# HKUST-KnowComp/DummyNode4GraphLearning

Hardware: AMD Instinct MI355X
Metric: edges/sec fwd+bwd on dummy-augmented RGIN conv (higher is better)
Workload: dtype bf16; 1 GPU; config5: RGINLayer(256,256,R=16,basis,relu) fwd+bwd, ONE global batch of 32768 graphs cut by parallel.shard_graphs over 1 GPU(s) (rank 0: N=1015808, E=3997696), SI dummy augmentation; global_edges=3997696, parallelism=dp1, rows_P=3112960, grad_bucket_bytes=2491904, hip_graph=True, sub_batches=1

## Files before the change

dummynode4graphlearning_amd/csrc/dn_chain_wgrad.hip:

```cpp
#include "dn_common.h"
#include "dn_internal.h"
#include "../../include/dn_hip.h"

namespace {

typedef __bf16 bf16_t;

constexpr int kH = 256;
constexpr int kTile = 64;
constexpr int kKC = 32;
constexpr int kThreads = 256;
constexpr int kAld = kTile + 2;

__device__ __forceinline__ double bf16_to_f64(bf16_t v) { return (double)(float)v; }

__device__ __forceinline__ bf16_t f64_to_bf16(double d) {
    float f = (float)d;
    if ((double)f != d && f == f && fabsf(f) < __builtin_huge_valf()) {
        uint32_t u = __float_as_uint(f);
        if (fabs((double)f) > fabs(d)) u -= 1u;
        f = __uint_as_float(u | 1u);
    }
    return (bf16_t)f;
}

__global__ __launch_bounds__(kThreads) void chain_combine_products_kernel(const float* __restrict__ M, const bf16_t* __restrict__ W1,
                                                                          const bf16_t* __restrict__ Wc,
                                                                          const bf16_t* __restrict__ Wc_loop, int32_t R,
                                                                          bf16_t* __restrict__ dWc, double* __restrict__ part) {
    __shared__ __attribute__((aligned(16))) double As[kKC * kAld];
    __shared__ __attribute__((aligned(16))) double Bs[kKC * kTile];
    const int tid = threadIdx.x, ty = tid >> 4, tx = tid & 15;
    const int m0 = (int)(blockIdx.x >> 2) * kTile, n0 = (int)(blockIdx.x & 3) * kTile;
    const int r = (int)blockIdx.y, kind = (int)blockIdx.z;
    const float* Mr = M + (size_t)r * kH * kH;
    const bf16_t* B = kind == 0 ? W1 : (r < R ? Wc + (size_t)r * kH * kH : Wc_loop);
    double acc[4][4];
#pragma unroll
    for (int i = 0; i < 4; ++i)
#pragma unroll
        for (int j = 0; j < 4; ++j) acc[i][j] = 0.0;
    float ra[8];
    bf16_t rb[8];
    auto fetch = [&](int kc) __attribute__((always_inline)) {
#pragma unroll
        for (int s = 0; s < 8; ++s) {
            if (kind == 0) ra[s] = Mr[(size_t)(m0 + (tid >> 5) + 8 * s) * kH + kc + (tid & 31)];
            else ra[s] = Mr[(size_t)(kc + (tid >> 6) + 4 * s) * kH + m0 + (tid & 63)];
            rb[s] = B[(size_t)(kc + (tid >> 6) + 4 * s) * kH + n0 + (tid & 63)];
        }
    };
    fetch(0);
    for (int kc = 0; kc < kH; kc += kKC) {
#pragma unroll
        for (int s = 0; s < 8; ++s) {
            if (kind == 0) As[(tid & 31) * kAld + (tid >> 5) + 8 * s] = (double)ra[s];
            else As[((tid >> 6) + 4 * s) * kAld + (tid & 63)] = (double)ra[s];
            Bs[((tid >> 6) + 4 * s) * kTile + (tid & 63)] = bf16_to_f64(rb[s]);
        }
        if (kc + kKC < kH) fetch(kc + kKC);
        __syncthreads();
#pragma unroll 8
        for (int k = 0; k < kKC; ++k) {
            const double2 a01 = *reinterpret_cast<const double2*>(&As[k * kAld + 4 * ty]);
            const double2 a23 = *reinterpret_cast<const double2*>(&As[k * kAld + 4 * ty + 2]);
            const double2 b01 = *reinterpret_cast<const double2*>(&Bs[k * kTile + 4 * tx]);
            const double2 b23 = *reinterpret_cast<const double2*>(&Bs[k * kTile + 4 * tx + 2]);
            const double a[4] = {a01.x, a01.y, a23.x, a23.y}, b[4] = {b01.x, b01.y, b23.x, b23.y};
#pragma unroll
            for (int i = 0; i < 4; ++i)
#pragma unroll
                for (int j = 0; j < 4; ++j) acc[i][j] = fma(a[i], b[j], acc[i][j]);
        }
        __syncthreads();
    }
#pragma unroll
    for (int i = 0; i < 4; ++i)
#pragma unroll
        for (int j = 0; j < 4; ++j) {
            const size_t o = (size_t)r * kH * kH + (size_t)(m0 + 4 * ty + i) * kH + n0 + 4 * tx + j;
            if (kind == 0) dWc[o] = f64_to_bf16(acc[i][j]);
            else part[o] = acc[i][j];
        }
}

__global__ __launch_bounds__(kH) void chain_combine_finish_kernel(const double* __restrict__ part, const float* __restrict__ c,
                                                                  const bf16_t* __restrict__ W1, const bf16_t* __restrict__ bias,
                                                                  int32_t R, bf16_t* __restrict__ dW1, bf16_t* __restrict__ db,
                                                                  bf16_t* __restrict__ db1) {
    const int h = threadIdx.x, j = (int)blockIdx.x;
    if (j < kH) {
        double sum = 0.0;
        for (int r = 0; r <= R; ++r) sum += part[(size_t)r * kH * kH + (size_t)j * kH + h];
        if (bias) sum = fma((double)c[j], bf16_to_f64(bias[h]), sum);
        dW1[(size_t)j * kH + h] = f64_to_bf16(sum);
        return;
    }
    if (db) {
        double sum = 0.0;
        for (int jj = 0; jj < kH; ++jj) sum = fma((double)c[jj], bf16_to_f64(W1[(size_t)jj * kH + h]), sum);
        db[h] = f64_to_bf16(sum);
    }
    if (db1) db1[h] = (bf16_t)c[h];
}

}

extern "C" int dn_layer_chain_dgrad_bf16(const void* G1, const void* W_kn, int64_t N, int32_t H, const int32_t* tiles, int64_t num_tiles,
                                         void* G0, void* seg_sums, dn_stream_t stream) {
    DN_REQUIRE(H == 256, "dn_layer_chain_dgrad: unsupported width %d (256 only)", H);
    DN_REQUIRE(N >= 0 && N < 0x7fffffffLL && num_tiles >= 0 && num_tiles < 0x7fffffffLL, "dn_layer_chain_dgrad: bad sizes");
    if (num_tiles == 0) return DN_OK;
    DN_REQUIRE(G1 && W_kn && tiles && G0 && seg_sums, "dn_layer_chain_dgrad: NULL pointer");
    DN_REQUIRE((reinterpret_cast<uintptr_t>(G1) | reinterpret_cast<uintptr_t>(W_kn) | reinterpret_cast<uintptr_t>(tiles) |
                reinterpret_cast<uintptr_t>(G0) | reinterpret_cast<uintptr_t>(seg_sums)) % 16 == 0, "dn_layer_chain_dgrad: unaligned pointer");
    return dn_internal::launch_transform_ring256_seg(G1, W_kn, tiles, num_tiles, G0, seg_sums, (hipStream_t)stream);
}

extern "C" size_t dn_layer_chain_wgrad_combine_workspace_bytes(int64_t R, int32_t H) {
    return R >= 0 && H > 0 ? (size_t)(R + 1) * (size_t)H * (size_t)H * sizeof(double) : 0;
}

extern "C" int dn_layer_chain_wgrad_combine(const float* M, const float* c, const void* W1, const void* Wc, const void* Wc_loop,
                                            const void* bias, int64_t R, int32_t H, void* dWc, void* db, void* dW1, void* db1,
                                            void* workspace, size_t workspace_bytes, dn_stream_t stream) {
    DN_REQUIRE(H == 256, "dn_layer_chain_wgrad_combine: unsupported width %d (256 only)", H);
    DN_REQUIRE(R >= 0 && R < 65535, "dn_layer_chain_wgrad_combine: bad relation count");
    DN_REQUIRE(M && c && W1 && Wc_loop && dWc && dW1 && workspace && (Wc || R == 0), "dn_layer_chain_wgrad_combine: NULL pointer");
    DN_REQUIRE(workspace_bytes >= dn_layer_chain_wgrad_combine_workspace_bytes(R, H), "dn_layer_chain_wgrad_combine: workspace too small");
    DN_REQUIRE((reinterpret_cast<uintptr_t>(M) | reinterpret_cast<uintptr_t>(workspace)) % 16 == 0,
               "dn_layer_chain_wgrad_combine: unaligned pointer");
    hipStream_t st = (hipStream_t)stream;
    double* part = (double*)workspace;
    hipLaunchKernelGGL(chain_combine_products_kernel, dim3((kH / kTile) * (kH / kTile), (unsigned)(R + 1), 2), dim3(kThreads), 0, st, M,
                       (const bf16_t*)W1, (const bf16_t*)Wc, (const bf16_t*)Wc_loop, (int32_t)R, (bf16_t*)dWc, part);
    DN_CHECK_LAUNCH();
    hipLaunchKernelGGL(chain_combine_finish_kernel, dim3(kH + 1), dim3(kH), 0, st, (const double*)part, c, (const bf16_t*)W1,
                       (const bf16_t*)bias, (int32_t)R, (bf16_t*)dW1, (bf16_t*)db, (bf16_t*)db1);
    DN_CHECK_LAUNCH();
    return DN_OK;
}
```

Before: 1.398 billion edges/s.

## Fuse chain wgrad combine into one FP64 MFMA kernel without workspace

```diff
diff --git a/dummynode4graphlearning_amd/csrc/dn_chain_wgrad.hip b/dummynode4graphlearning_amd/csrc/dn_chain_wgrad.hip
--- a/dummynode4graphlearning_amd/csrc/dn_chain_wgrad.hip
+++ b/dummynode4graphlearning_amd/csrc/dn_chain_wgrad.hip
@@ -7,10 +7,12 @@
 typedef __bf16 bf16_t;
 
 constexpr int kH = 256;
-constexpr int kTile = 64;
-constexpr int kKC = 32;
+constexpr int kT = 16;
 constexpr int kThreads = 256;
-constexpr int kAld = kTile + 2;
+constexpr int kW1Blocks = (kH / kT) * (kH / kT);
+constexpr int kWcBlocksPerRel = (kH / kT) * (kH / (4 * kT));
+
+typedef double f64x4 __attribute__((ext_vector_type(4)));
 
 __device__ __forceinline__ double bf16_to_f64(bf16_t v) { return (double)(float)v; }
 
@@ -24,81 +26,116 @@
     return (bf16_t)f;
 }
 
-__global__ __launch_bounds__(kThreads) void chain_combine_products_kernel(const float* __restrict__ M, const bf16_t* __restrict__ W1,
-                                                                          const bf16_t* __restrict__ Wc,
-                                                                          const bf16_t* __restrict__ Wc_loop, int32_t R,
-                                                                          bf16_t* __restrict__ dWc, double* __restrict__ part) {
-    __shared__ __attribute__((aligned(16))) double As[kKC * kAld];
-    __shared__ __attribute__((aligned(16))) double Bs[kKC * kTile];
-    const int tid = threadIdx.x, ty = tid >> 4, tx = tid & 15;
-    const int m0 = (int)(blockIdx.x >> 2) * kTile, n0 = (int)(blockIdx.x & 3) * kTile;
-    const int r = (int)blockIdx.y, kind = (int)blockIdx.z;
-    const float* Mr = M + (size_t)r * kH * kH;
-    const bf16_t* B = kind == 0 ? W1 : (r < R ? Wc + (size_t)r * kH * kH : Wc_loop);
-    double acc[4][4];
+__device__ __forceinline__ f64x4 mfma_f64(double a, double b, f64x4 acc) { return __builtin_amdgcn_mfma_f64_16x16x4f64(a, b, acc, 0, 0, 0); }
+
+constexpr int kU = 8;
+
+__device__ __forceinline__ f64x4 chain_rows(const float* __restrict__ Ap, const bf16_t* __restrict__ Bp, int steps, f64x4 acc) {
+    float a0[kU], a1[kU];
+    bf16_t b0[kU], b1[kU];
+    auto load = [&](float (&a)[kU], bf16_t (&b)[kU], int s) __attribute__((always_inline)) {
 #pragma unroll
-    for (int i = 0; i < 4; ++i)
-#pragma unroll
-        for (int j = 0; j < 4; ++j) acc[i][j] = 0.0;
-    float ra[8];
-    bf16_t rb[8];
-    auto fetch = [&](int kc) __attribute__((always_inline)) {
-#pragma unroll
-        for (int s = 0; s < 8; ++s) {
-            if (kind == 0) ra[s] = Mr[(size_t)(m0 + (tid >> 5) + 8 * s) * kH + kc + (tid & 31)];
-            else ra[s] = Mr[(size_t)(kc + (tid >> 6) + 4 * s) * kH + m0 + (tid & 63)];
-            rb[s] = B[(size_t)(kc + (tid >> 6) + 4 * s) * kH + n0 + (tid & 63)];
+        for (int u = 0; u < kU; ++u) {
+            a[u] = Ap[(size_t)(s + u) * 4 * kH];
+            b[u] = Bp[(size_t)(s + u) * 4 * kH];
         }
     };
-    fetch(0);
-    for (int kc = 0; kc < kH; kc += kKC) {
+    auto mma = [&](const float (&a)[kU], const bf16_t (&b)[kU]) __attribute__((always_inline)) {
 #pragma unroll
-        for (int s = 0; s < 8; ++s) {
-            if (kind == 0) As[(tid & 31) * kAld + (tid >> 5) + 8 * s] = (double)ra[s];
-            else As[((tid >> 6) + 4 * s) * kAld + (tid & 63)] = (double)ra[s];
-            Bs[((tid >> 6) + 4 * s) * kTile + (tid & 63)] = bf16_to_f64(rb[s]);
-        }
-        if (kc + kKC < kH) fetch(kc + kKC);
-        __syncthreads();
-#pragma unroll 8
-        for (int k = 0; k < kKC; ++k) {
-            const double2 a01 = *reinterpret_cast<const double2*>(&As[k * kAld + 4 * ty]);
-            const double2 a23 = *reinterpret_cast<const double2*>(&As[k * kAld + 4 * ty + 2]);
-            const double2 b01 = *reinterpret_cast<const double2*>(&Bs[k * kTile + 4 * tx]);
-            const double2 b23 = *reinterpret_cast<const double2*>(&Bs[k * kTile + 4 * tx + 2]);
-            const double a[4] = {a01.x, a01.y, a23.x, a23.y}, b[4] = {b01.x, b01.y, b23.x, b23.y};
-#pragma unroll
-            for (int i = 0; i < 4; ++i)
-#pragma unroll
-                for (int j = 0; j < 4; ++j) acc[i][j] = fma(a[i], b[j], acc[i][j]);
-        }
-        __syncthreads();
+        for (int u = 0; u < kU; ++u) acc = mfma_f64((double)a[u], bf16_to_f64(b[u]), acc);
+    };
+    if (steps <= 0) return acc;
+    load(a0, b0, 0);
+    for (int s = 0; s < steps; s += 2 * kU) {
+        load(a1, b1, s + kU);
+        mma(a0, b0);
+        if (s + 2 * kU < steps) load(a0, b0, s + 2 * kU);
+        mma(a1, b1);
     }
-#pragma unroll
-    for (int i = 0; i < 4; ++i)
-#pragma unroll
-        for (int j = 0; j < 4; ++j) {
-            const size_t o = (size_t)r * kH * kH + (size_t)(m0 + 4 * ty + i) * kH + n0 + 4 * tx + j;
-            if (kind == 0) dWc[o] = f64_to_bf16(acc[i][j]);
-            else part[o] = acc[i][j];
-        }
+    return acc;
 }
 
-__global__ __launch_bounds__(kH) void chain_combine_finish_kernel(const double* __restrict__ part, const float* __restrict__ c,
-                                                                  const bf16_t* __restrict__ W1, const bf16_t* __restrict__ bias,
-                                                                  int32_t R, bf16_t* __restrict__ dW1, bf16_t* __restrict__ db,
-                                                                  bf16_t* __restrict__ db1) {
-    const int h = threadIdx.x, j = (int)blockIdx.x;
-    if (j < kH) {
-        double sum = 0.0;
-        for (int r = 0; r <= R; ++r) sum += part[(size_t)r * kH * kH + (size_t)j * kH + h];
-        if (bias) sum = fma((double)c[j], bf16_to_f64(bias[h]), sum);
-        dW1[(size_t)j * kH + h] = f64_to_bf16(sum);
+__global__ __launch_bounds__(kThreads) void chain_combine_mfma_kernel(const float* __restrict__ M, const float* __restrict__ c,
+                                                                      const bf16_t* __restrict__ W1, const bf16_t* __restrict__ Wc,
+                                                                      const bf16_t* __restrict__ Wc_loop, const bf16_t* __restrict__ bias,
+                                                                      int32_t R, bf16_t* __restrict__ dWc, bf16_t* __restrict__ db,
+                                                                      bf16_t* __restrict__ dW1, bf16_t* __restrict__ db1) {
+    __shared__ double red[3][4][64];
+    const int tid = threadIdx.x, lane = tid & 63, wave = tid >> 6, li = lane & 15, lk = lane >> 4;
+    const int b = (int)blockIdx.x;
+    if (b < kW1Blocks) {
+        const int m0 = (2 * (b & 7) + ((b >> 3) & 1)) * kT, n0 = (b >> 4) * kT;
+        const int rows = (R + 1) * (kH / 4), row0 = wave * rows, loop0 = R * kH;
+        const int rows_wc = min(max(loop0 - row0, 0), rows);
+        const float* Ap = M + (size_t)(row0 + lk) * kH + m0 + li;
+        f64x4 acc = {0.0, 0.0, 0.0, 0.0};
+        if (rows_wc > 0) acc = chain_rows(Ap, Wc + (size_t)(row0 + lk) * kH + n0 + li, rows_wc / 4, acc);
+        if (rows_wc < rows)
+            acc = chain_rows(Ap + (size_t)rows_wc * kH, Wc_loop + (size_t)(row0 + rows_wc - loop0 + lk) * kH + n0 + li, (rows - rows_wc) / 4, acc);
+        if (wave)
+#pragma unroll
+            for (int v = 0; v < 4; ++v) red[wave - 1][v][lane] = acc[v];
+        __syncthreads();
+        if (wave) return;
+#pragma unroll
+        for (int v = 0; v < 4; ++v) {
+            const int j = m0 + lk + 4 * v, h = n0 + li;
+            double sum = ((acc[v] + red[0][v][lane]) + red[1][v][lane]) + red[2][v][lane];
+            if (bias) sum = fma((double)c[j], bf16_to_f64(bias[h]), sum);
+            dW1[(size_t)j * kH + h] = f64_to_bf16(sum);
+        }
         return;
     }
+    const int t = b - kW1Blocks;
+    if (t < (R + 1) * kWcBlocksPerRel) {
+        const int id = (t >> 5) * 8 + (t & 7), r = id >> 4, m0 = (id & 15) * kT, n0 = ((t >> 3) & 3) * 4 * kT + wave * kT;
+        const float* Ap = M + ((size_t)r * kH + m0 + li) * kH + 4 * lk;
+        const bf16_t* Bp = W1 + (size_t)(4 * lk) * kH + n0 + li;
+        f64x4 acc = {0.0, 0.0, 0.0, 0.0};
+        float4 a0[2], a1[2];
+        bf16_t b0[2][4], b1[2][4];
+        auto load = [&](float4 (&a)[2], bf16_t (&bb)[2][4], int kc) __attribute__((always_inline)) {
+#pragma unroll
+            for (int u = 0; u < 2; ++u) {
+                a[u] = *reinterpret_cast<const float4*>(Ap + kc + 16 * u);
+#pragma unroll
+                for (int s = 0; s < 4; ++s) bb[u][s] = Bp[(size_t)(kc + 16 * u + s) * kH];
+            }
+        };
+        auto mma = [&](const float4 (&a)[2], const bf16_t (&bb)[2][4]) __attribute__((always_inline)) {
+#pragma unroll
+            for (int u = 0; u < 2; ++u) {
+                acc = mfma_f64((double)a[u].x, bf16_to_f64(bb[u][0]), acc);
+                acc = mfma_f64((double)a[u].y, bf16_to_f64(bb[u][1]), acc);
+                acc = mfma_f64((double)a[u].z, bf16_to_f64(bb[u][2]), acc);
+                acc = mfma_f64((double)a[u].w, bf16_to_f64(bb[u][3]), acc);
+            }
+        };
+        load(a0, b0, 0);
+        for (int kc = 0; kc < kH; kc += 64) {
+            load(a1, b1, kc + 32);
+            mma(a0, b0);
+            if (kc + 64 < kH) load(a0, b0, kc + 64);
+            mma(a1, b1);
+        }
+#pragma unroll
+        for (int v = 0; v < 4; ++v)
+            dWc[((size_t)r * kH + m0 + lk + 4 * v) * kH + n0 + li] = f64_to_bf16(acc[v]);
+        return;
+    }
+    const int h = tid;
+    double* cs = &red[0][0][0];
+    cs[h] = (double)c[h];
+    __syncthreads();
     if (db) {
         double sum = 0.0;
-        for (int jj = 0; jj < kH; ++jj) sum = fma((double)c[jj], bf16_to_f64(W1[(size_t)jj * kH + h]), sum);
+        for (int j0 = 0; j0 < kH; j0 += 32) {
+            bf16_t w[32];
+#pragma unroll
+            for (int u = 0; u < 32; ++u) w[u] = W1[(size_t)(j0 + u) * kH + h];
+#pragma unroll
+            for (int u = 0; u < 32; ++u) sum = fma(cs[j0 + u], bf16_to_f64(w[u]), sum);
+        }
         db[h] = f64_to_bf16(sum);
     }
     if (db1) db1[h] = (bf16_t)c[h];
@@ -118,25 +155,22 @@
 }
 
 extern "C" size_t dn_layer_chain_wgrad_combine_workspace_bytes(int64_t R, int32_t H) {
-    return R >= 0 && H > 0 ? (size_t)(R + 1) * (size_t)H * (size_t)H * sizeof(double) : 0;
+    (void)R, (void)H;
+    return 0;
 }
 
 extern "C" int dn_layer_chain_wgrad_combine(const float* M, const float* c, const void* W1, const void* Wc, const void* Wc_loop,
                                             const void* bias, int64_t R, int32_t H, void* dWc, void* db, void* dW1, void* db1,
                                             void* workspace, size_t workspace_bytes, dn_stream_t stream) {
+    (void)workspace, (void)workspace_bytes;
     DN_REQUIRE(H == 256, "dn_layer_chain_wgrad_combine: unsupported width %d (256 only)", H);
     DN_REQUIRE(R >= 0 && R < 65535, "dn_layer_chain_wgrad_combine: bad relation count");
-    DN_REQUIRE(M && c && W1 && Wc_loop && dWc && dW1 && workspace && (Wc || R == 0), "dn_layer_chain_wgrad_combine: NULL pointer");
-    DN_REQUIRE(workspace_bytes >= dn_layer_chain_wgrad_combine_workspace_bytes(R, H), "dn_layer_chain_wgrad_combine: workspace too small");
-    DN_REQUIRE((reinterpret_cast<uintptr_t>(M) | reinterpret_cast<uintptr_t>(workspace)) % 16 == 0,
-               "dn_layer_chain_wgrad_combine: unaligned pointer");
-    hipStream_t st = (hipStream_t)stream;
-    double* part = (double*)workspace;
-    hipLaunchKernelGGL(chain_combine_products_kernel, dim3((kH / kTile) * (kH / kTile), (unsigned)(R + 1), 2), dim3(kThreads), 0, st, M,
-                       (const bf16_t*)W1, (const bf16_t*)Wc, (const bf16_t*)Wc_loop, (int32_t)R, (bf16_t*)dWc, part);
-    DN_CHECK_LAUNCH();
-    hipLaunchKernelGGL(chain_combine_finish_kernel, dim3(kH + 1), dim3(kH), 0, st, (const double*)part, c, (const bf16_t*)W1,
-                       (const bf16_t*)bias, (int32_t)R, (bf16_t*)dW1, (bf16_t*)db, (bf16_t*)db1);
+    DN_REQUIRE(M && c && W1 && Wc_loop && dWc && dW1 && (Wc || R == 0), "dn_layer_chain_wgrad_combine: NULL pointer");
+    DN_REQUIRE(reinterpret_cast<uintptr_t>(M) % 16 == 0, "dn_layer_chain_wgrad_combine: unaligned pointer");
+    const unsigned blocks = (unsigned)(kW1Blocks + (R + 1) * kWcBlocksPerRel + 1);
+    hipLaunchKernelGGL(chain_combine_mfma_kernel, dim3(blocks), dim3(kThreads), 0, (hipStream_t)stream, M, c, (const bf16_t*)W1,
+                       (const bf16_t*)Wc, (const bf16_t*)Wc_loop, (const bf16_t*)bias, (int32_t)R, (bf16_t*)dWc, (bf16_t*)db,
+                       (bf16_t*)dW1, (bf16_t*)db1);
     DN_CHECK_LAUNCH();
     return DN_OK;
 }
```

New measurement: 1.404 billion edges/s, median of 6. No clear change (+0.4%).
